# PaoloRibeca/KPop

Measured on AMD Instinct MI355X. Metric: sequences/sec end-to-end count->twist->distance, k=12, 100k x 150bp, higher is better.
Workload: dtype f64; 1 GPU; 100000 reads x 150 bp per GPU, k=12 DNA-ds, 65 class vectors, euclidean, metric powers(1,1,2); read_len=150, k=12, n_dims=64, n_classes=65, class_len=30000, twister=8390656 canonical k-mers x 64 dims, f64, synthetic, replicated on every GPU, reads_per_gpu=100000

## Files before the change

kpop_amd/csrc/class_set.hip:

```cpp
#include <algorithm>

#include "common.h"
#include "space_ops.h"
#include "distance_routes.h"

namespace kpop {

constexpr int kClassRows = 64;
constexpr int kClassGroup = 8;
constexpr int kClassFlight = 4;
constexpr uint32_t kClassSetMinRows = 128;

template <int KIND>
__global__ __launch_bounds__(256) void class_set_prepare_kernel(const double *__restrict__ m1, uint32_t r1, uint32_t n_dims, uint32_t dp,
                                                                const double *__restrict__ metric, double p, const double *__restrict__ norms1,
                                                                bool divide, double *__restrict__ n1_out, double *__restrict__ cls) {
  const uint32_t lane = threadIdx.x & 63u, i = blockIdx.x * 4u + (threadIdx.x >> 6);
  if (i >= r1) return;
  const bool in = lane < n_dims;
  const double el = in ? m1[(uint64_t)i * n_dims + lane] : 0.0, mc = in ? metric[lane] : 0.0;
  double nv = 1.0;
  if (divide) {
    if (norms1) {
      nv = norms1[i];
    } else {
      const double t = component<KIND>(el, mc, p);
      double acc = 0.0;
#pragma unroll
      for (int c = 0; c < 64; ++c)
        acc = __dadd_rn(acc, __hiloint2double(__builtin_amdgcn_readlane(__double2hiint(t), c), __builtin_amdgcn_readlane(__double2loint(t), c)));
      nv = scale_distance<KIND>(acc, p);
      nv = (nv == 0.0) ? 1.0 : nv;
      if (n1_out && lane == 0) n1_out[i] = nv;
    }
  }
  if (lane < dp) {
    cls[(uint64_t)i * 2u * dp + lane] = in ? (divide ? __ddiv_rn(el, nv) : el) : 0.0;
    cls[(uint64_t)i * 2u * dp + dp + lane] = mc;
  }
}

template <int KIND, int DP, int NC>
__device__ __forceinline__ void class_set_chain(const double (&x)[DP], const double *__restrict__ cls, uint32_t i, double p, double *stage) {
  double acc[NC];
#pragma unroll
  for (int k = 0; k < NC; ++k) acc[k] = 0.0;
  const double *__restrict__ a = cls + (uint64_t)i * (2 * DP);
  const double *__restrict__ metp = a + DP;
#pragma unroll
  for (int g = 0; g < DP; g += kClassGroup) {
#pragma unroll
    for (int d = 0; d < kClassGroup; ++d) {
      const double mc = metp[g + d];
#pragma unroll
      for (int k = 0; k < NC; ++k) {
        const double diff = __dsub_rn(a[k * (2 * DP) + g + d], x[g + d]);
        acc[k] = __dadd_rn(acc[k], component<KIND>(diff, mc, p));
      }
    }
  }
#pragma unroll
  for (int k = 0; k < NC; ++k) stage[i + k] = scale_distance<KIND>(acc[k], p);
}

template <int KIND, int DP, bool DIVIDE>
__global__ __launch_bounds__(256, DP == 64 ? 3 : 4) void class_set_distance_kernel(const double *__restrict__ cls,
                                                                                  uint32_t r1, const double *__restrict__ m2, uint32_t r2,
                                                                                  uint32_t n_dims, double p, double *__restrict__ n2,
                                                                                  double *__restrict__ out, uint32_t n_full, uint32_t tail_parts) {
  extern __shared__ __attribute__((aligned(16))) double class_lds[];
  constexpr int LD = DP + 1;
  constexpr int kPer = kClassRows * DP / 256;
  double *tile = class_lds;
  uint32_t rb = blockIdx.x, part = 0, parts = 1;
  if (blockIdx.x >= n_full) {
    const uint32_t t = blockIdx.x - n_full;
    rb = n_full + t / tail_parts;
    part = t % tail_parts;
    parts = tail_parts;
  }
  const uint32_t row0 = rb * (uint32_t)kClassRows;
  const uint32_t nrows = min((uint32_t)kClassRows, r2 - row0);
  {
    double pre[kPer];
#pragma unroll
    for (int u = 0; u < kPer; ++u) {
      const uint32_t e = threadIdx.x + 256u * u, i = e / DP, c = e % DP;
      pre[u] = m2[(uint64_t)min(row0 + i, r2 - 1u) * n_dims + min(c, n_dims - 1u)];
    }
#pragma unroll
    for (int u = 0; u < kPer; ++u) {
      const uint32_t e = threadIdx.x + 256u * u, i = e / DP, c = e % DP;
      tile[i * LD + c] = (i < nrows && c < n_dims) ? pre[u] : 0.0;
    }
  }
  __syncthreads();
  if (DIVIDE) {
    if (threadIdx.x < (uint32_t)kClassRows) {
      const double *row = tile + threadIdx.x * LD;
      const double *__restrict__ metp = cls + DP;
      double acc = 0.0;
#pragma unroll
      for (int c = 0; c < DP; ++c) acc = __dadd_rn(acc, component<KIND>(row[c], metp[c], p));
      double nv = scale_distance<KIND>(acc, p);
      nv = (nv == 0.0) ? 1.0 : nv;
      tile[threadIdx.x * LD + DP] = nv;
      if (threadIdx.x < nrows && part == 0) n2[row0 + threadIdx.x] = nv;
    }
    __syncthreads();
#pragma unroll
    for (int u = 0; u < kPer; ++u) {
      const uint32_t e = threadIdx.x + 256u * u, i = e / DP, c = e % DP;
      if (c < n_dims) tile[i * LD + c] = __ddiv_rn(tile[i * LD + c], tile[i * LD + DP]);
    }
    __syncthreads();
  }
  const uint32_t lane = threadIdx.x & 63u;
  double x[DP];
#pragma unroll
  for (int c = 0; c < DP; ++c) x[c] = tile[lane * LD + c];
  __syncthreads();
  const uint32_t wv = __builtin_amdgcn_readfirstlane(threadIdx.x >> 6);
  const uint32_t slices = 4u * parts, u = 4u * part + wv;
  const uint32_t c_hi = (u + 1u) * r1 / slices;
  const uint32_t RS = r1 | 1u;
  double *stage = class_lds + lane * RS;
  uint32_t i = u * r1 / slices;
  for (; i + kClassFlight <= c_hi; i += kClassFlight) class_set_chain<KIND, DP, kClassFlight>(x, cls, i, p, stage);
  for (; i < c_hi; ++i) class_set_chain<KIND, DP, 1>(x, cls, i, p, stage);
  __syncthreads();
  const uint32_t b_lo = part * r1 / parts, bw = (part + 1u) * r1 / parts - b_lo;
  if (bw == 0) return;
  const uint32_t total = nrows * bw, dj = 256u / bw, di = 256u % bw;
  double *__restrict__ dst = out + (uint64_t)row0 * r1 + b_lo;
  const double *src = class_lds + b_lo;
  uint32_t j = threadIdx.x / bw, ii = threadIdx.x % bw;
  for (uint32_t e = threadIdx.x; e < total; e += 256u) {
    dst[(uint64_t)j * r1 + ii] = src[j * RS + ii];
    j += dj;
    ii += di;
    if (ii >= bw) {
      ii -= bw;
      ++j;
    }
  }
}

static uint32_t class_set_padded_dims(uint32_t n_dims) { return n_dims <= 8 ? 8u : n_dims <= 16 ? 16u : n_dims <= 32 ? 32u : 64u; }

bool class_set_applies(int kind, uint32_t r1, uint32_t r2, uint32_t n_dims, uint64_t room_doubles) {
  const int mode = ctx().tune_class_set;
  if (mode == 0 || (kind != KPOP_EUCLIDEAN && kind != KPOP_COSINE)) return false;
  if (n_dims == 0 || n_dims > 64 || r1 < 1 || r1 >= 128 || r2 < 1 || r2 >= (1u << 30)) return false;
  const uint64_t dp = class_set_padded_dims(n_dims);
  if (2u * (uint64_t)r1 * dp > room_doubles) return false;
  return mode == 2 || r2 >= kClassSetMinRows;
}

template <int KIND, int DP>
static int launch_class_set_dp(const double *cls, uint32_t r1, const double *m2, uint32_t r2, uint32_t n_dims, double p,
                               bool divide, double *n2, double *out, hipStream_t st) {
  const uint32_t slots = (uint32_t)ctx().n_cus * (DP == 64 ? 3u : 4u), blocks = div_up(r2, kClassRows);
  const uint32_t tail = blocks % slots;
  uint32_t parts = 1;
  if (tail) parts = tail * 8u <= slots ? 8u : tail * 4u <= slots ? 4u : tail * 2u <= slots ? 2u : 1u;
  parts = std::max(1u, std::min(parts, r1 / 4u));
  const uint32_t n_full = parts > 1 ? blocks - tail : blocks;
  const dim3 grid(n_full + (blocks - n_full) * parts), block(256);
  const size_t lds = sizeof(double) * kClassRows * std::max<size_t>(DP + 1, r1 | 1u);
  if (divide) class_set_distance_kernel<KIND, DP, true><<<grid, block, lds, st>>>(cls, r1, m2, r2, n_dims, p, n2, out, n_full, parts);
  else class_set_distance_kernel<KIND, DP, false><<<grid, block, lds, st>>>(cls, r1, m2, r2, n_dims, p, n2, out, n_full, parts);
  KPOP_LAUNCH_CHECK();
  return 0;
}

template <int KIND>
static int launch_class_set_kind(const double *m1, uint32_t r1, const double *norms1, double *n1_out, const double *m2, uint32_t r2, double *n2,
                                 uint32_t n_dims, const double *metric, double p, bool divide, double *room, double *out, hipStream_t st) {
  const uint32_t dp = class_set_padded_dims(n_dims);
  double *cls = room;
  class_set_prepare_kernel<KIND><<<dim3(div_up(r1, 4)), dim3(256), 0, st>>>(m1, r1, n_dims, dp, metric, p, norms1, divide, n1_out, cls);
  KPOP_LAUNCH_CHECK();
  switch (dp) {
    case 8: return launch_class_set_dp<KIND, 8>(cls, r1, m2, r2, n_dims, p, divide, n2, out, st);
    case 16: return launch_class_set_dp<KIND, 16>(cls, r1, m2, r2, n_dims, p, divide, n2, out, st);
    case 32: return launch_class_set_dp<KIND, 32>(cls, r1, m2, r2, n_dims, p, divide, n2, out, st);
    default: return launch_class_set_dp<KIND, 64>(cls, r1, m2, r2, n_dims, p, divide, n2, out, st);
  }
}

int launch_class_set_distance(int kind, const double *m1, uint32_t r1, const double *norms1, double *n1_out, const double *m2, uint32_t r2, double *n2,
                              uint32_t n_dims, const double *metric, double p, bool divide, double *room, double *out, hipStream_t st) {
  if (kind == KPOP_EUCLIDEAN) return launch_class_set_kind<KPOP_EUCLIDEAN>(m1, r1, norms1, n1_out, m2, r2, n2, n_dims, metric, p, divide, room, out, st);
  return launch_class_set_kind<KPOP_COSINE>(m1, r1, norms1, n1_out, m2, r2, n2, n_dims, metric, p, divide, room, out, st);
}

}
```

Baseline: 82.56 million sequences/sec.

## Software-pipeline class operand fetches with double-buffered groups and rebalance flights

Rewrites the class-distance inner loop to double-buffer operand loads, fetching the next group of class coefficients while the current group is computed, with schedule barriers pinning the order. It also stores the metric once instead of per class row, staggers the wave-to-slice mapping by row block, and splits the class work into 4-wide flights plus a 5-wide or small remainder flight. Scalar parameters are parked in vector registers and recovered after the main loop to lower SGPR pressure. The inline asm and schedule barriers add complexity and could raise register use or block other compiler scheduling.

```diff
diff --git a/kpop_amd/csrc/class_set.hip b/kpop_amd/csrc/class_set.hip
--- a/kpop_amd/csrc/class_set.hip
+++ b/kpop_amd/csrc/class_set.hip
@@ -7,8 +7,8 @@
 namespace kpop {
 
 constexpr int kClassRows = 64;
-constexpr int kClassGroup = 8;
-constexpr int kClassFlight = 4;
+constexpr int kClassGroup = 4;
+constexpr int kClassGroupWide = 2;
 constexpr uint32_t kClassSetMinRows = 128;
 
 template <int KIND>
@@ -35,32 +35,92 @@
     }
   }
   if (lane < dp) {
-    cls[(uint64_t)i * 2u * dp + lane] = in ? (divide ? __ddiv_rn(el, nv) : el) : 0.0;
-    cls[(uint64_t)i * 2u * dp + dp + lane] = mc;
-  }
-}
-
-template <int KIND, int DP, int NC>
-__device__ __forceinline__ void class_set_chain(const double (&x)[DP], const double *__restrict__ cls, uint32_t i, double p, double *stage) {
-  double acc[NC];
-#pragma unroll
-  for (int k = 0; k < NC; ++k) acc[k] = 0.0;
-  const double *__restrict__ a = cls + (uint64_t)i * (2 * DP);
-  const double *__restrict__ metp = a + DP;
-#pragma unroll
-  for (int g = 0; g < DP; g += kClassGroup) {
-#pragma unroll
-    for (int d = 0; d < kClassGroup; ++d) {
-      const double mc = metp[g + d];
-#pragma unroll
-      for (int k = 0; k < NC; ++k) {
-        const double diff = __dsub_rn(a[k * (2 * DP) + g + d], x[g + d]);
-        acc[k] = __dadd_rn(acc[k], component<KIND>(diff, mc, p));
-      }
-    }
-  }
-#pragma unroll
-  for (int k = 0; k < NC; ++k) stage[i + k] = scale_distance<KIND>(acc[k], p);
+    cls[(1u + i) * dp + lane] = in ? (divide ? __ddiv_rn(el, nv) : el) : 0.0;
+    if (i == 0) cls[lane] = mc;
+  }
+}
+
+template <int NC, int G>
+struct ClassOperands {
+  double a[NC][G], m[G];
+};
+
+template <int DP, int NC, int G>
+__device__ __forceinline__ void class_set_fetch(ClassOperands<NC, G> &o, const double *__restrict__ cls, const double *__restrict__ a, int g) {
+#pragma unroll
+  for (int k = 0; k < NC; ++k)
+#pragma unroll
+    for (int d = 0; d < G; ++d) o.a[k][d] = a[k * DP + g + d];
+#pragma unroll
+  for (int d = 0; d < G; ++d) o.m[d] = cls[g + d];
+}
+
+template <int KIND, int DP, int NC, int G>
+__device__ __forceinline__ void class_set_group(const ClassOperands<NC, G> &o, const double (&x)[DP], int g, double p, double (&acc)[NC]) {
+#pragma unroll
+  for (int d = 0; d < G; ++d) {
+#pragma unroll
+    for (int k = 0; k < NC; ++k) {
+      const double diff = __dsub_rn(o.a[k][d], x[g + d]);
+      acc[k] = __dadd_rn(acc[k], component<KIND>(diff, o.m[d], p));
+    }
+  }
+}
+
+template <int NC, int G>
+__device__ __forceinline__ uint32_t class_set_landed(const ClassOperands<NC, G> &o, uint32_t next, double &acc) {
+  asm volatile("" : "+s"(next), "+v"(acc) : "s"(__double2loint(o.m[0])));
+  return next;
+}
+
+template <int KIND, int DP, int NC, int G>
+__device__ __forceinline__ void class_set_flights(const double (&x)[DP], const double *__restrict__ cls, uint32_t i, uint32_t n, double p,
+                                                  double *stage) {
+  static_assert(DP % (2 * G) == 0, "the groups alternate between two sets of operands");
+  ClassOperands<NC, G> s0, s1;
+  uint32_t a = (1u + i) * DP;
+  double *st = stage + i;
+  class_set_fetch<DP, NC, G>(s0, cls, cls + a, 0);
+  for (;;) {
+    --n;
+    const uint32_t nxt = n ? a + NC * DP : a;
+    double acc[NC];
+#pragma unroll
+    for (int k = 0; k < NC; ++k) acc[k] = 0.0;
+#pragma unroll
+    for (int g = 0; g < DP; g += 2 * G) {
+      a = class_set_landed(s0, a, acc[0]);
+      class_set_fetch<DP, NC, G>(s1, cls, cls + a, g + G);
+      __builtin_amdgcn_sched_barrier(0);
+      class_set_group<KIND, DP, NC, G>(s0, x, g, p, acc);
+      __builtin_amdgcn_sched_barrier(0);
+      a = class_set_landed(s1, g + 2 * G < DP ? a : nxt, acc[0]);
+      class_set_fetch<DP, NC, G>(s0, cls, cls + a, g + 2 * G < DP ? g + 2 * G : 0);
+      __builtin_amdgcn_sched_barrier(0);
+      class_set_group<KIND, DP, NC, G>(s1, x, g + G, p, acc);
+      __builtin_amdgcn_sched_barrier(0);
+    }
+#pragma unroll
+    for (int k = 0; k < NC; ++k) st[k] = scale_distance<KIND>(acc[k], p);
+    st += NC;
+    if (n == 0) break;
+  }
+}
+
+__device__ __forceinline__ uint32_t class_set_aside(uint32_t s) {
+  uint32_t v;
+  asm("v_mov_b32 %0, %1" : "=v"(v) : "s"(s));
+  return v;
+}
+
+__device__ __forceinline__ void class_set_block(uint32_t bx, uint32_t n_full, uint32_t tail_parts, uint32_t &rb, uint32_t &part, uint32_t &parts) {
+  rb = bx, part = 0, parts = 1;
+  if (bx >= n_full) {
+    const uint32_t t = bx - n_full;
+    rb = n_full + t / tail_parts;
+    part = t % tail_parts;
+    parts = tail_parts;
+  }
 }
 
 template <int KIND, int DP, bool DIVIDE>
@@ -72,13 +132,8 @@
   constexpr int LD = DP + 1;
   constexpr int kPer = kClassRows * DP / 256;
   double *tile = class_lds;
-  uint32_t rb = blockIdx.x, part = 0, parts = 1;
-  if (blockIdx.x >= n_full) {
-    const uint32_t t = blockIdx.x - n_full;
-    rb = n_full + t / tail_parts;
-    part = t % tail_parts;
-    parts = tail_parts;
-  }
+  uint32_t rb, part, parts;
+  class_set_block(blockIdx.x, n_full, tail_parts, rb, part, parts);
   const uint32_t row0 = rb * (uint32_t)kClassRows;
   const uint32_t nrows = min((uint32_t)kClassRows, r2 - row0);
   {
@@ -98,7 +153,7 @@
   if (DIVIDE) {
     if (threadIdx.x < (uint32_t)kClassRows) {
       const double *row = tile + threadIdx.x * LD;
-      const double *__restrict__ metp = cls + DP;
+      const double *__restrict__ metp = cls;
       double acc = 0.0;
 #pragma unroll
       for (int c = 0; c < DP; ++c) acc = __dadd_rn(acc, component<KIND>(row[c], metp[c], p));
@@ -120,23 +175,39 @@
 #pragma unroll
   for (int c = 0; c < DP; ++c) x[c] = tile[lane * LD + c];
   __syncthreads();
-  const uint32_t wv = __builtin_amdgcn_readfirstlane(threadIdx.x >> 6);
-  const uint32_t slices = 4u * parts, u = 4u * part + wv;
-  const uint32_t c_hi = (u + 1u) * r1 / slices;
+  const uint32_t k_bx = class_set_aside(blockIdx.x), k_n_full = class_set_aside(n_full), k_tail_parts = class_set_aside(tail_parts),
+                 k_r1 = class_set_aside(r1), k_r2 = class_set_aside(r2);
+  const uint32_t wv = threadIdx.x >> 6;
+  const uint32_t slices = 4u * parts, u = 4u * part + ((wv + rb) & 3u);
+  const uint32_t c_lo_v = u * r1 / slices, c_hi_v = (u + 1u) * r1 / slices;
   const uint32_t RS = r1 | 1u;
   double *stage = class_lds + lane * RS;
-  uint32_t i = u * r1 / slices;
-  for (; i + kClassFlight <= c_hi; i += kClassFlight) class_set_chain<KIND, DP, kClassFlight>(x, cls, i, p, stage);
-  for (; i < c_hi; ++i) class_set_chain<KIND, DP, 1>(x, cls, i, p, stage);
+  uint32_t i = __builtin_amdgcn_readfirstlane(c_lo_v);
+  {
+    const uint32_t n = c_hi_v - c_lo_v, q = n / 4u, r = n % 4u, n4 = __builtin_amdgcn_readfirstlane(q >= r ? q - r : q);
+    if (n4) class_set_flights<KIND, DP, 4, kClassGroup>(x, cls, i, n4, p, stage);
+    i = __builtin_amdgcn_readfirstlane(c_lo_v + 4u * (q >= r ? q - r : q));
+  }
+  const uint32_t left = __builtin_amdgcn_readfirstlane(c_hi_v) - i;
+  if (left >= 5u) class_set_flights<KIND, DP, 5, kClassGroupWide>(x, cls, i, left / 5u, p, stage);
+  else if (left == 3u) class_set_flights<KIND, DP, 3, kClassGroup>(x, cls, i, 1u, p, stage);
+  else if (left == 2u) class_set_flights<KIND, DP, 2, kClassGroup>(x, cls, i, 1u, p, stage);
+  else if (left == 1u) class_set_flights<KIND, DP, 1, kClassGroup>(x, cls, i, 1u, p, stage);
   __syncthreads();
-  const uint32_t b_lo = part * r1 / parts, bw = (part + 1u) * r1 / parts - b_lo;
+  const uint32_t r1_6 = __builtin_amdgcn_readfirstlane(k_r1);
+  uint32_t rb6, part6, parts6;
+  class_set_block(__builtin_amdgcn_readfirstlane(k_bx), __builtin_amdgcn_readfirstlane(k_n_full), __builtin_amdgcn_readfirstlane(k_tail_parts),
+                  rb6, part6, parts6);
+  const uint32_t row6 = rb6 * (uint32_t)kClassRows, nrows6 = min((uint32_t)kClassRows, __builtin_amdgcn_readfirstlane(k_r2) - row6);
+  const uint32_t b_lo = part6 * r1_6 / parts6, bw = (part6 + 1u) * r1_6 / parts6 - b_lo;
   if (bw == 0) return;
-  const uint32_t total = nrows * bw, dj = 256u / bw, di = 256u % bw;
-  double *__restrict__ dst = out + (uint64_t)row0 * r1 + b_lo;
+  const uint32_t RS6 = r1_6 | 1u;
+  const uint32_t total = nrows6 * bw, dj = 256u / bw, di = 256u % bw;
+  double *__restrict__ dst = out + (uint64_t)row6 * r1_6 + b_lo;
   const double *src = class_lds + b_lo;
   uint32_t j = threadIdx.x / bw, ii = threadIdx.x % bw;
   for (uint32_t e = threadIdx.x; e < total; e += 256u) {
-    dst[(uint64_t)j * r1 + ii] = src[j * RS + ii];
+    dst[(uint64_t)j * r1_6 + ii] = src[j * RS6 + ii];
     j += dj;
     ii += di;
     if (ii >= bw) {
```

Result: slower. 81.44 million sequences/sec (-1.3%).

## Double-buffer class row fetches via scalar constant loads in distance chain

Applied to the files above, without the earlier changes.

Class vectors and metric are now read as 4-wide double groups through a volatile constant-address-space pointer, so they go through the scalar load path. The next group is prefetched into a second buffer while the current one is computed, with explicit waitcnt and sched barriers enforcing the order. The group size drops from 8 to 4, and the per-dimension arithmetic is split into separate sub, square, scale and add passes. This removes the generic component call and asserts that Minkowski is never used here. The hand-written waitcnt, inline asm and volatile loads may constrain the compiler and cost registers.

```diff
diff --git a/kpop_amd/csrc/class_set.hip b/kpop_amd/csrc/class_set.hip
--- a/kpop_amd/csrc/class_set.hip
+++ b/kpop_amd/csrc/class_set.hip
@@ -7,7 +7,7 @@
 namespace kpop {
 
 constexpr int kClassRows = 64;
-constexpr int kClassGroup = 8;
+constexpr int kClassGroup = 4;
 constexpr int kClassFlight = 4;
 constexpr uint32_t kClassSetMinRows = 128;
 
@@ -40,24 +40,54 @@
   }
 }
 
+typedef double class_group __attribute__((ext_vector_type(4), aligned(8)));
+typedef const volatile __attribute__((address_space(4))) class_group *class_ptr;
+static_assert(kClassGroup == 4, "a class_group is kClassGroup doubles");
+
+template <int DP, int NC>
+__device__ __forceinline__ void class_set_fetch(class_group (&buf)[NC + 1], class_ptr a, int g) {
+#pragma unroll
+  for (int k = 0; k < NC; ++k) buf[k] = a[(k * (2 * DP) + g) / kClassGroup];
+  buf[NC] = a[(DP + g) / kClassGroup];
+}
+
+template <int NC>
+__device__ __forceinline__ void class_set_arrived(class_ptr &a, double (&acc)[NC]) {
+  __builtin_amdgcn_s_waitcnt(0xc07f);
+  static_assert(NC == kClassFlight || NC == 1, "the statement names every sum");
+  if constexpr (NC == 1) asm volatile("" : "+s"(a), "+v"(acc[0]));
+  else asm volatile("" : "+s"(a), "+v"(acc[0]), "+v"(acc[1]), "+v"(acc[2]), "+v"(acc[3]));
+  __builtin_amdgcn_sched_barrier(0);
+}
+
 template <int KIND, int DP, int NC>
 __device__ __forceinline__ void class_set_chain(const double (&x)[DP], const double *__restrict__ cls, uint32_t i, double p, double *stage) {
   double acc[NC];
 #pragma unroll
   for (int k = 0; k < NC; ++k) acc[k] = 0.0;
-  const double *__restrict__ a = cls + (uint64_t)i * (2 * DP);
-  const double *__restrict__ metp = a + DP;
+  class_ptr a = (class_ptr)(cls + (uint64_t)i * (2 * DP));
+  class_group buf[2][NC + 1];
+  class_set_fetch<DP, NC>(buf[0], a, 0);
 #pragma unroll
   for (int g = 0; g < DP; g += kClassGroup) {
+    const int b = (g / kClassGroup) & 1;
+    class_set_arrived<NC>(a, acc);
+    if (g + kClassGroup < DP) class_set_fetch<DP, NC>(buf[b ^ 1], a, g + kClassGroup);
+    __builtin_amdgcn_sched_barrier(0);
 #pragma unroll
     for (int d = 0; d < kClassGroup; ++d) {
-      const double mc = metp[g + d];
-#pragma unroll
-      for (int k = 0; k < NC; ++k) {
-        const double diff = __dsub_rn(a[k * (2 * DP) + g + d], x[g + d]);
-        acc[k] = __dadd_rn(acc[k], component<KIND>(diff, mc, p));
-      }
-    }
+      static_assert(KIND != KPOP_MINKOWSKI, "component<KIND> is diff *. diff *. m");
+      double t[NC];
+#pragma unroll
+      for (int k = 0; k < NC; ++k) t[k] = __dsub_rn(buf[b][k][d], x[g + d]);
+#pragma unroll
+      for (int k = 0; k < NC; ++k) t[k] = __dmul_rn(t[k], t[k]);
+#pragma unroll
+      for (int k = 0; k < NC; ++k) t[k] = __dmul_rn(t[k], buf[b][NC][d]);
+#pragma unroll
+      for (int k = 0; k < NC; ++k) acc[k] = __dadd_rn(acc[k], t[k]);
+    }
+    __builtin_amdgcn_sched_barrier(0);
   }
 #pragma unroll
   for (int k = 0; k < NC; ++k) stage[i + k] = scale_distance<KIND>(acc[k], p);
```

Result: no change. 82.47 million sequences/sec before, 82.80 million sequences/sec after, median of 4 (+0.4%).
